# OpenGVLab/VisionLLM

Measured on NVIDIA H100. Metric: img_text_pairs_per_sec_fwd_1024px_256tok, higher is better.
Workload: dtype bf16

## Files before the change

visionllm_b200/csrc/gemm.cu:

```cuda
#include "common.cuh"
#include "tc_common.cuh"
#include "vllm_b200.h"

namespace {

constexpr int BM = 128, BK = 64, THREADS = 384, CONSUMER_WARPS = 8, CONSUMER_THREADS = CONSUMER_WARPS * 32;
constexpr int A_BYTES = BM * BK * 2;
constexpr int EPI_PITCH = 128 + 16;
constexpr int EPI_WARP_BYTES = 16 * EPI_PITCH;

enum { ACT_NONE = 0, ACT_GELU = 1, ACT_RELU = 2, ACT_SILU = 3, ACT_SWIGLU = 4, ACT_QUICKGELU = 5 };

struct GemmArgs {
  int M, N, K;
  void* C; int ldc;
  const __nv_bfloat16* bias; const __nv_bfloat16* colscale; const __nv_bfloat16* residual; int ldr;
  int act; int out_f32;
  const unsigned char* row_keep;
  int tiles_m, tiles_n;
  int group_m;
  int a_seg_kb, a_seg_rows;
  int sc_rows;
  void* sc_dst[8];
  uint32_t* sc_flag[8];
  int a_mn, b_mn;
  int bt_rows, causal;
};

struct TilePlan { int skip, kb0, kb1, b_row_off, k_off; };
__device__ __forceinline__ TilePlan plan_tile(const GemmArgs& g, int m0, int n0, int rows_per_tile, int num_kb) {
  TilePlan p{0, 0, num_kb, 0, 0};
  if (g.bt_rows) {
    const int bh = m0 / g.bt_rows, ml = m0 - bh * g.bt_rows;
    p.b_row_off = bh * g.N;
    p.k_off = bh * g.K;
    if (g.causal == 1 && n0 >= ml + rows_per_tile) p.skip = 1;
    if (g.causal == 2) p.kb0 = ml / BK;
    if (g.causal == 3) { const int e = (ml + rows_per_tile + BK - 1) / BK; p.kb1 = e < num_kb ? e : num_kb; }
  }
  return p;
}

template <int BN> struct Cfg {
  static constexpr int B_BYTES = BN * BK * 2;
  static constexpr int STAGE_BYTES = A_BYTES + B_BYTES;
  static constexpr int STAGES = BN == 256 ? 4 : 6;
  static constexpr int SMEM = STAGES * STAGE_BYTES + 1024  + 256  + 2 * BN * 4  +
                              CONSUMER_WARPS * EPI_WARP_BYTES ;
};

__device__ __forceinline__ float gelu_erf(float x) { return 0.5f * x * (1.f + erff(x * 0.70710678118654752f)); }
__device__ __forceinline__ float silu(float x) { return x / (1.f + __expf(-x)); }

__device__ __forceinline__ void tile_coords(int t, int tiles_m, int tiles_n, int group_m, int& tm, int& tn) {
  const int per_group = group_m * tiles_n;
  const int group = t / per_group;
  const int first = group * group_m;
  const int gsz = min(group_m, tiles_m - first);
  const int in = t - group * per_group;
  tm = first + in % gsz;
  tn = in / gsz;
}

template <int BN, int TA, int TB>
__device__ __forceinline__ void mma_kblock(float (&acc)[BN / 2], uint32_t sa, uint32_t sb, bool first_kb) {
  const uint64_t adesc = TA ? tc::wgmma_desc_sw128(sa, 8192, 1024) : tc::wgmma_desc_sw128(sa, 16, 1024);
  const uint64_t bdesc = TB ? tc::wgmma_desc_sw128(sb, 8192, 1024) : tc::wgmma_desc_sw128(sb, 16, 1024);
  constexpr uint64_t astep = TA ? 128 : 2, bstep = TB ? 128 : 2;
#pragma unroll
  for (int k = 0; k < BK / 16; ++k) {
    if constexpr (BN == 256)
      tc::wgmma_m64n256k16_ss<TA, TB>(acc, adesc + astep * k, bdesc + bstep * k, !(first_kb && k == 0));
    else
      tc::wgmma_m64n128k16_ss<TA, TB>(acc, adesc + astep * k, bdesc + bstep * k, !(first_kb && k == 0));
  }
}

enum { EPI_BF16 = 0, EPI_GENERAL = 1, EPI_SCATTER = 2 };

template <int BN, int TA, int TB, int EPI>
__global__ void __launch_bounds__(THREADS, 1)
gemm_bf16_wgmma_kernel(const __grid_constant__ CUtensorMap tmap_a, const __grid_constant__ CUtensorMap tmap_b,
                       const GemmArgs g) {
  using C_ = Cfg<BN>;
  constexpr int STAGES = C_::STAGES;
  extern __shared__ uint8_t smem_raw[];
  const uint32_t smem_base = (tc::smem_u32(smem_raw) + 1023u) & ~1023u;
  uint8_t* smem_gen = smem_raw + (smem_base - tc::smem_u32(smem_raw));
  const uint32_t bar_base = smem_base + STAGES * C_::STAGE_BYTES;
  auto full_bar = [&](int s) { return bar_base + 8 * s; };
  auto empty_bar = [&](int s) { return bar_base + 8 * (STAGES + s); };
  float* s_bias = reinterpret_cast<float*>(smem_gen + STAGES * C_::STAGE_BYTES + 256);
  float* s_scale = s_bias + BN;
  uint8_t* s_epi = reinterpret_cast<uint8_t*>(s_scale + BN);

  const int warp = threadIdx.x >> 5, lane = threadIdx.x & 31;
  const int n_tiles = g.tiles_m * g.tiles_n;
  const int num_kb = (g.K + BK - 1) / BK;

  if (warp == 0 && lane == 0) {
    tc::tma_prefetch_desc(&tmap_a);
    tc::tma_prefetch_desc(&tmap_b);
  }
  if (warp == 1 && lane == 0) {
    for (int s = 0; s < STAGES; ++s) { tc::mbar_init(full_bar(s), 1); tc::mbar_init(empty_bar(s), CONSUMER_WARPS); }
    tc::mbar_fence_init();
  }
  __syncthreads();

  if (warp < 4) {
    tc::reg_dealloc<40>();
    if (warp == 0 && tc::elect_one()) {
      int stage = 0; uint32_t phase = 0;
      for (int t = blockIdx.x; t < n_tiles; t += gridDim.x) {
        int tm, tn; tile_coords(t, g.tiles_m, g.tiles_n, g.group_m, tm, tn);
        const TilePlan tp = plan_tile(g, tm * BM, tn * BN, BM, num_kb);
        if (tp.skip) continue;
        const int bt_m0 = g.bt_rows ? (tm * BM) / g.bt_rows * g.bt_rows : 0;
        const int row_a = tm * BM - (TA ? bt_m0 : 0);
        const int row_b = tn * BN + (TB ? 0 : tp.b_row_off);
        const int ka_off = TA ? tp.k_off : 0, kb_off = TB ? tp.k_off : 0;
        for (int kb = tp.kb0; kb < tp.kb1; ++kb) {
          tc::mbar_wait(empty_bar(stage), phase ^ 1);
          const uint32_t sa = smem_base + stage * C_::STAGE_BYTES, sb = sa + A_BYTES;
          int ka = kb * BK + ka_off, ra = row_a;
          if (g.a_seg_kb) {
            const int seg = kb / g.a_seg_kb;
            ka = (kb - seg * g.a_seg_kb) * BK;
            ra = row_a + seg * g.a_seg_rows;
          }
          tc::mbar_arrive_expect_tx(full_bar(stage), C_::STAGE_BYTES);
          if constexpr (TA) {
            for (int h = 0; h < BM / 64; ++h) tc::tma_load_2d(sa + h * 8192, &tmap_a, full_bar(stage), ra + 64 * h, ka);
          } else {
            tc::tma_load_2d(sa, &tmap_a, full_bar(stage), ka, ra);
          }
          if constexpr (TB) {
            for (int h = 0; h < BN / 64; ++h)
              tc::tma_load_2d(sb + h * 8192, &tmap_b, full_bar(stage), row_b + 64 * h, kb * BK + kb_off);
          } else {
            tc::tma_load_2d(sb, &tmap_b, full_bar(stage), kb * BK, row_b);
          }
          if (++stage == STAGES) { stage = 0; phase ^= 1; }
        }
      }
    }
    return;
  }

  tc::reg_alloc<232>();
  const int wg = (warp - 4) >> 2;
  const int et = threadIdx.x - 128;
  const int frag_row = wg * 64 + (warp & 3) * 16 + (lane >> 2), frag_col = 2 * (lane & 3);
  const bool swiglu = EPI == EPI_GENERAL && g.act == ACT_SWIGLU;
  int stage = 0; uint32_t phase = 0;
  float acc[BN / 2];
  for (int t = blockIdx.x; t < n_tiles; t += gridDim.x) {
    int tm, tn; tile_coords(t, g.tiles_m, g.tiles_n, g.group_m, tm, tn);
    const TilePlan tp = plan_tile(g, tm * BM, tn * BN, BM, num_kb);
    if (tp.skip) continue;
    const int n0 = tn * BN;
    if (et < BN) {
      const int col = n0 + et;
      s_bias[et] = (g.bias && col < g.N) ? __bfloat162float(g.bias[col]) : 0.f;
      s_scale[et] = (g.colscale && col < g.N) ? __bfloat162float(g.colscale[col]) : 1.f;
    }
    int prev_stage = -1;
    for (int kb = tp.kb0; kb < tp.kb1; ++kb) {
      tc::mbar_wait(full_bar(stage), phase);
      const uint32_t sa = smem_base + stage * C_::STAGE_BYTES + wg * 8192, sb = smem_base + stage * C_::STAGE_BYTES + A_BYTES;
      const bool first = kb == tp.kb0;
      tc::acc_fence(acc);
      tc::wgmma_fence();
      mma_kblock<BN, TA, TB>(acc, sa, sb, first);
      tc::wgmma_commit();
      tc::wgmma_wait<1>();
      if (prev_stage >= 0 && lane == 0) tc::mbar_arrive(empty_bar(prev_stage));
      prev_stage = stage;
      if (++stage == STAGES) { stage = 0; phase ^= 1; }
    }
    tc::wgmma_wait<0>();
    tc::acc_fence(acc);
    if (lane == 0) tc::mbar_arrive(empty_bar(prev_stage));
    tc::named_bar_sync(1, CONSUMER_THREADS);

    auto math = [&](int row, int c, float& v0, float& v1) {
      const int col = n0 + c;
      v0 += s_bias[c]; v1 += s_bias[c + 1];
      if (g.act == ACT_GELU) { v0 = gelu_erf(v0); v1 = gelu_erf(v1); }
      else if (g.act == ACT_RELU) { v0 = fmaxf(v0, 0.f); v1 = fmaxf(v1, 0.f); }
      else if (g.act == ACT_SILU) { v0 = silu(v0); v1 = silu(v1); }
      else if (g.act == ACT_QUICKGELU) { v0 = v0 / (1.f + __expf(-1.702f * v0)); v1 = v1 / (1.f + __expf(-1.702f * v1)); }
      v0 *= s_scale[c]; v1 *= s_scale[c + 1];
      if (row >= g.M) return;
      if (g.residual) {
        const __nv_bfloat16* rp = g.residual + (size_t)row * g.ldr + col;
        if (col + 1 < g.N) {
          const float2 f = __bfloat1622float2(*reinterpret_cast<const __nv_bfloat162*>(rp));
          v0 += f.x; v1 += f.y;
        } else {
          v0 += __bfloat162float(rp[0]);
        }
      }
      if (g.row_keep && !g.row_keep[row]) { v0 = 0.f; v1 = 0.f; }
    };
    auto out_row = [&](int row) -> __nv_bfloat16* {
      if constexpr (EPI != EPI_SCATTER) return reinterpret_cast<__nv_bfloat16*>(g.C) + (size_t)row * g.ldc;
      const int d = row / g.sc_rows;
      return reinterpret_cast<__nv_bfloat16*>(g.sc_dst[d]) + (size_t)(row - d * g.sc_rows) * g.ldc;
    };
    auto emit = [&](int row, int c, float v0, float v1) {
      const int col = n0 + c;
      if (row >= g.M || col >= g.N) return;
      if (swiglu) {
        const int oc = col >> 1;
        float o = silu(v0 + s_bias[c]) * (v1 + s_bias[c + 1]);
        if (g.residual) o += __bfloat162float(g.residual[(size_t)row * g.ldr + oc]);
        reinterpret_cast<__nv_bfloat16*>(g.C)[(size_t)row * g.ldc + oc] = __float2bfloat16(o);
        return;
      }
      math(row, c, v0, v1);
      const bool pair = col + 1 < g.N;
      if (g.out_f32) {
        float* cp = reinterpret_cast<float*>(g.C) + (size_t)row * g.ldc + col;
        if (pair) *reinterpret_cast<float2*>(cp) = make_float2(v0, v1); else cp[0] = v0;
        return;
      }
      __nv_bfloat16* cp = out_row(row) + col;
      if (pair) *reinterpret_cast<__nv_bfloat162*>(cp) = __floats2bfloat162_rn(v0, v1); else cp[0] = __float2bfloat16(v0);
    };
    const int row0 = tm * BM + frag_row;
    const int warp_row0 = tm * BM + wg * 64 + (warp & 3) * 16;
    uint8_t* my_stage = s_epi + (warp - 4) * EPI_WARP_BYTES;
#pragma unroll
    for (int ch = 0; ch < BN / 64; ++ch) {
      const int c0 = ch * 64;
      if (n0 + c0 >= g.N) break;
      if constexpr (EPI == EPI_GENERAL) {
#pragma unroll
        for (int j = 8 * ch; j < 8 * ch + 8; ++j) {
          const int c = 8 * j + frag_col;
          emit(row0, c, acc[4 * j], acc[4 * j + 1]);
          emit(row0 + 8, c, acc[4 * j + 2], acc[4 * j + 3]);
        }
      } else {
#pragma unroll
        for (int j = 8 * ch; j < 8 * ch + 8; ++j) {
          const int c = 8 * j + frag_col;
          float a0 = acc[4 * j], a1 = acc[4 * j + 1], b0 = acc[4 * j + 2], b1 = acc[4 * j + 3];
          math(row0, c, a0, a1);
          math(row0 + 8, c, b0, b1);
          const int off = (8 * (j - 8 * ch) + frag_col) * 2;
          *reinterpret_cast<__nv_bfloat162*>(my_stage + (lane >> 2) * EPI_PITCH + off) = __floats2bfloat162_rn(a0, a1);
          *reinterpret_cast<__nv_bfloat162*>(my_stage + ((lane >> 2) + 8) * EPI_PITCH + off) = __floats2bfloat162_rn(b0, b1);
        }
        __syncwarp();
#pragma unroll
        for (int it = 0; it < 4; ++it) {
          const int rr = it * 4 + (lane >> 3), piece = lane & 7;
          const uint4 val = *reinterpret_cast<const uint4*>(my_stage + rr * EPI_PITCH + piece * 16);
          if (warp_row0 + rr < g.M) *reinterpret_cast<uint4*>(out_row(warp_row0 + rr) + n0 + c0 + piece * 8) = val;
        }
        __syncwarp();
      }
    }
    if constexpr (EPI == EPI_SCATTER) {
      __threadfence_system();
      __syncwarp();
      if (lane == 0 && warp_row0 < g.M)
        asm volatile("red.release.sys.global.add.u32 [%0], %1;" ::"l"(g.sc_flag[warp_row0 / g.sc_rows]), "r"(1u) : "memory");
    }
    tc::named_bar_sync(1, CONSUMER_THREADS);
  }
}

int g_sm_limit = 0, g_scatter_sm_limit = 0;

int g_gemm_variant = VLLM_GEMM_DEFAULT;

using KernelFn = void (*)(const CUtensorMap, const CUtensorMap, const GemmArgs);

template <int BN, int TA, int TB>
KernelFn pick_epilogue(const GemmArgs& g) {
  if (g.sc_rows) {
    if constexpr (BN == 256 && !TA && !TB) return gemm_bf16_wgmma_kernel<BN, TA, TB, EPI_SCATTER>;
    return nullptr;
  }
  if (g.act == ACT_SWIGLU || g.out_f32 || g.N % 64) return gemm_bf16_wgmma_kernel<BN, TA, TB, EPI_GENERAL>;
  return gemm_bf16_wgmma_kernel<BN, TA, TB, EPI_BF16>;
}
template <int BN>
KernelFn pick_kernel(const GemmArgs& g) {
  if (g.a_mn) return g.b_mn ? pick_epilogue<BN, 1, 1>(g) : pick_epilogue<BN, 1, 0>(g);
  return g.b_mn ? pick_epilogue<BN, 0, 1>(g) : pick_epilogue<BN, 0, 0>(g);
}

template <int BN>
int launch_gemm(const void* A, int lda, const void* B, int ldb, GemmArgs g, cudaStream_t st, long long a_rows = -1,
                int a_cols = -1) {
  using C_ = Cfg<BN>;
  CUtensorMap ta, tb;
  const uint64_t nb = g.bt_rows ? (uint64_t)(g.M / g.bt_rows) : 1;
  const uint64_t m_local = g.bt_rows ? (uint64_t)g.bt_rows : (uint64_t)g.M;
  int rc = g.a_mn ? vllm_make_tmap_bf16(&ta, A, nb * (uint64_t)g.K, m_local, (uint64_t)lda, 64)
                  : vllm_make_tmap_bf16(&ta, A, (uint64_t)(a_rows < 0 ? g.M : a_rows),
                                        (uint64_t)(a_cols < 0 ? g.K : a_cols), (uint64_t)lda, BM);
  if (rc) return rc;
  rc = g.b_mn ? vllm_make_tmap_bf16(&tb, B, nb * (uint64_t)g.K, (uint64_t)g.N, (uint64_t)ldb, 64)
              : vllm_make_tmap_bf16(&tb, B, nb * (uint64_t)g.N, (uint64_t)g.K, (uint64_t)ldb, BN);
  if (rc) return rc;
  g.tiles_m = (g.M + BM - 1) / BM;
  g.tiles_n = (g.N + BN - 1) / BN;
  const int n_tiles = g.tiles_m * g.tiles_n;
  int sms = vllm_num_sms();
  const int limit = g.sc_rows ? (g_scatter_sm_limit > 0 ? g_scatter_sm_limit : g_sm_limit) : g_sm_limit;
  if (limit > 0 && limit < sms) sms = limit;
  const int ctas = sms < n_tiles ? sms : n_tiles;
  g.group_m = 8;
  const KernelFn kern = pick_kernel<BN>(g);
  if (!kern) return VLLM_EUNSUPPORTED;
  const cudaError_t e = vllm_smem_optin(kern, C_::SMEM);
  if (e != cudaSuccess) return (int)e;
  kern<<<ctas, THREADS, C_::SMEM, st>>>(ta, tb, g);
  VLLM_CHECK_LAUNCH();
  return VLLM_OK;
}

bool wide_by_shape(const GemmArgs& g) {
  return !g.a_mn && !g.b_mn && !g.bt_rows && !g.a_seg_kb && g.N <= 4096 && g.K >= 3072;
}

int launch_gemm_auto(const void* A, int lda, const void* B, int ldb, const GemmArgs& g, cudaStream_t st, long long a_rows = -1,
                     int a_cols = -1) {
  const bool wide = g.sc_rows || g_gemm_variant == VLLM_GEMM_WIDE_TILE ||
                    (g_gemm_variant == VLLM_GEMM_DEFAULT && wide_by_shape(g));
  return wide ? launch_gemm<256>(A, lda, B, ldb, g, st, a_rows, a_cols) : launch_gemm<128>(A, lda, B, ldb, g, st, a_rows, a_cols);
}

}

extern "C" {

int vllm_gemm_set_variant(int v) {
  if (v != VLLM_GEMM_DEFAULT && v != VLLM_GEMM_WIDE_TILE && v != VLLM_GEMM_NARROW_TILE) return VLLM_EINVAL;
  g_gemm_variant = v;
  return VLLM_OK;
}
int vllm_gemm_set_sm_limit(int all_gemms, int scatter_gemm) {
  if (all_gemms < 0 || scatter_gemm < 0) return VLLM_EINVAL;
  g_sm_limit = all_gemms; g_scatter_sm_limit = scatter_gemm;
  return VLLM_OK;
}

static int gemm_bf16_common(const void* A, int lda, const void* B, int ldb, void* C, int ldc, int M, int N, int K,
                            const void* bias, const void* colscale, const void* residual, int ldr, int act, int out_f32,
                            const unsigned char* row_keep, void* stream);

int vllm_gemm_bf16(const void* A, int lda, const void* B, int ldb, void* C, int ldc, int M, int N, int K,
                   const void* bias, const void* colscale, const void* residual, int ldr, int act, int out_f32,
                   void* stream) {
  return gemm_bf16_common(A, lda, B, ldb, C, ldc, M, N, K, bias, colscale, residual, ldr, act, out_f32, nullptr, stream);
}

int vllm_gemm_bf16_rowmask(const void* A, int lda, const void* B, int ldb, void* C, int ldc, int M, int N, int K,
                           const void* bias, const void* colscale, const void* residual, int ldr, int act, int out_f32,
                           const unsigned char* row_keep, void* stream) {
  if (!row_keep || act == ACT_SWIGLU) return VLLM_EINVAL;
  return gemm_bf16_common(A, lda, B, ldb, C, ldc, M, N, K, bias, colscale, residual, ldr, act, out_f32, row_keep, stream);
}

static int gemm_bf16_common(const void* A, int lda, const void* B, int ldb, void* C, int ldc, int M, int N, int K,
                            const void* bias, const void* colscale, const void* residual, int ldr, int act, int out_f32,
                            const unsigned char* row_keep, void* stream) {
  if (M < 0 || N <= 0 || K <= 0 || lda < K || ldb < K) return VLLM_EINVAL;
  if (M == 0) return VLLM_OK;
  if (!A || !B || !C) return VLLM_EINVAL;
  if (act < 0 || act > ACT_QUICKGELU) return VLLM_EINVAL;
  const int n_out = act == ACT_SWIGLU ? N / 2 : N;
  if (act == ACT_SWIGLU && (N % 2 || out_f32 || colscale)) return VLLM_EUNSUPPORTED;
  if (ldc < n_out || (residual && ldr < n_out)) return VLLM_EINVAL;
  if (!vllm_aligned(A, 16) || !vllm_aligned(B, 16) || (lda % 8) || (ldb % 8)) return VLLM_EALIGN;
  const int celt = out_f32 ? 4 : 2;
  if (!vllm_aligned(C, 16) || ((size_t)ldc * celt) % 16 || (residual && (!vllm_aligned(residual, 16) || ldr % 8)))
    return VLLM_EALIGN;
  GemmArgs g{};
  g.M = M; g.N = N; g.K = K; g.C = C; g.ldc = ldc;
  g.bias = (const __nv_bfloat16*)bias; g.colscale = (const __nv_bfloat16*)colscale;
  g.residual = (const __nv_bfloat16*)residual; g.ldr = ldr; g.act = act; g.out_f32 = out_f32;
  g.row_keep = row_keep;
  cudaStream_t st = (cudaStream_t)stream;
  return launch_gemm_auto(A, lda, B, ldb, g, st);
}

int vllm_gemm_bf16_tn(const void* A, int lda, int a_mn_major, const void* B, int ldb, int b_mn_major, void* C, int ldc, int M,
                      int N, int K, int out_f32, void* stream) {
  if (M < 0 || N <= 0 || K <= 0) return VLLM_EINVAL;
  if (M == 0) return VLLM_OK;
  if (!A || !B || !C) return VLLM_EINVAL;
  if (lda < (a_mn_major ? M : K) || ldb < (b_mn_major ? N : K) || ldc < N) return VLLM_EINVAL;
  if (!vllm_aligned(A, 16) || !vllm_aligned(B, 16) || (lda % 8) || (ldb % 8)) return VLLM_EALIGN;
  if (!vllm_aligned(C, 16) || ((size_t)ldc * (out_f32 ? 4 : 2)) % 16) return VLLM_EALIGN;
  GemmArgs g{};
  g.M = M; g.N = N; g.K = K; g.C = C; g.ldc = ldc; g.out_f32 = out_f32;
  g.a_mn = a_mn_major ? 1 : 0; g.b_mn = b_mn_major ? 1 : 0;
  cudaStream_t st = (cudaStream_t)stream;
  return launch_gemm_auto(A, lda, B, ldb, g, st);
}

int vllm_gemm_bf16_batched(const void* A, int lda, int a_mn_major, const void* B, int ldb, int b_mn_major, void* C, int ldc,
                           int n_batch, int M, int N, int K, int causal, int out_f32, void* stream) {
  if (n_batch < 0 || M <= 0 || N <= 0 || K <= 0 || causal < 0 || causal > 3) return VLLM_EINVAL;
  if (causal >= 2 && K != M) return VLLM_EINVAL;
// ... 59 lines not shown
```

visionllm_b200/csrc/tc_common.cuh:

```cuda
#pragma once
#include <cuda.h>
#include <cuda_runtime.h>
#include <stdint.h>

namespace tc {

__device__ __forceinline__ uint32_t smem_u32(const void* p) {
  return static_cast<uint32_t>(__cvta_generic_to_shared(p));
}
__device__ __forceinline__ bool elect_one() {
  uint32_t pred = 0;
  asm volatile(
      "{\n\t.reg .pred P;\n\telect.sync _|P, 0xffffffff;\n\tselp.u32 %0, 1, 0, P;\n\t}\n"
      : "=r"(pred));
  return pred != 0;
}

__device__ __forceinline__ void mbar_init(uint32_t bar, uint32_t count) {
  asm volatile("mbarrier.init.shared::cta.b64 [%0], %1;" ::"r"(bar), "r"(count) : "memory");
}
__device__ __forceinline__ void mbar_fence_init() {
  asm volatile("fence.mbarrier_init.release.cluster;" ::: "memory");
}
__device__ __forceinline__ void mbar_arrive_expect_tx(uint32_t bar, uint32_t bytes) {
  asm volatile("mbarrier.arrive.expect_tx.shared::cta.b64 _, [%0], %1;" ::"r"(bar), "r"(bytes) : "memory");
}
__device__ __forceinline__ void mbar_arrive(uint32_t bar) {
  asm volatile("mbarrier.arrive.shared::cta.b64 _, [%0];" ::"r"(bar) : "memory");
}
__device__ __forceinline__ bool mbar_try_wait(uint32_t bar, uint32_t parity) {
  uint32_t ok;
  asm volatile(
      "{\n\t.reg .pred p;\n\tmbarrier.try_wait.parity.shared::cta.b64 p, [%1], %2;\n\tselp.u32 %0, 1, 0, p;\n\t}\n"
      : "=r"(ok)
      : "r"(bar), "r"(parity)
      : "memory");
  return ok != 0;
}
__device__ __forceinline__ void mbar_wait(uint32_t bar, uint32_t parity) {
  while (!mbar_try_wait(bar, parity)) {
  }
}
__device__ __forceinline__ void tma_prefetch_desc(const CUtensorMap* m) {
  asm volatile("prefetch.tensormap [%0];" ::"l"(reinterpret_cast<uint64_t>(m)) : "memory");
}
__device__ __forceinline__ void tma_load_2d(uint32_t dst, const CUtensorMap* m, uint32_t bar, int c0, int c1) {
  asm volatile(
      "cp.async.bulk.tensor.2d.shared::cluster.global.mbarrier::complete_tx::bytes [%0], [%1, {%3, %4}], [%2];" ::"r"(dst),
      "l"(reinterpret_cast<uint64_t>(m)), "r"(bar), "r"(c0), "r"(c1)
      : "memory");
}

template <int N> __device__ __forceinline__ void reg_dealloc() { asm volatile("setmaxnreg.dec.sync.aligned.u32 %0;" ::"n"(N)); }
template <int N> __device__ __forceinline__ void reg_alloc() { asm volatile("setmaxnreg.inc.sync.aligned.u32 %0;" ::"n"(N)); }
__device__ __forceinline__ void named_bar_sync(int id, int threads) {
  asm volatile("bar.sync %0, %1;" ::"r"(id), "r"(threads) : "memory");
}

__device__ __forceinline__ void wgmma_fence() { asm volatile("wgmma.fence.sync.aligned;" ::: "memory"); }
__device__ __forceinline__ void wgmma_commit() { asm volatile("wgmma.commit_group.sync.aligned;" ::: "memory"); }
template <int N> __device__ __forceinline__ void wgmma_wait() { asm volatile("wgmma.wait_group.sync.aligned %0;" ::"n"(N) : "memory"); }
template <int N> __device__ __forceinline__ void acc_fence(float (&d)[N]) {
#pragma unroll
  for (int i = 0; i < N; ++i) asm volatile("" : "+f"(d[i])::"memory");
}

template <int TA, int TB>
__device__ __forceinline__ void wgmma_m64n128k16_ss(float (&d)[64], uint64_t adesc, uint64_t bdesc, uint32_t accumulate) {
  asm volatile(
      "{\n\t.reg .pred p;\n\tsetp.ne.b32 p, %66, 0;\n\t"
      "wgmma.mma_async.sync.aligned.m64n128k16.f32.bf16.bf16 {"
      "%0, %1, %2, %3, %4, %5, %6, %7, %8, %9, %10, %11, %12, %13, %14, %15, %16, %17, %18, %19, %20, %21, "
      "%22, %23, %24, %25, %26, %27, %28, %29, %30, %31, %32, %33, %34, %35, %36, %37, %38, %39, %40, %41, "
      "%42, %43, %44, %45, %46, %47, %48, %49, %50, %51, %52, %53, %54, %55, %56, %57, %58, %59, %60, %61, "
      "%62, %63 "
      "}, %64, %65, p, 1, 1, %67, %68;\n\t}\n"
      : "+f"(d[0]), "+f"(d[1]), "+f"(d[2]), "+f"(d[3]), "+f"(d[4]), "+f"(d[5]), "+f"(d[6]), "+f"(d[7]),
        "+f"(d[8]), "+f"(d[9]), "+f"(d[10]), "+f"(d[11]), "+f"(d[12]), "+f"(d[13]), "+f"(d[14]), "+f"(d[15]),
        "+f"(d[16]), "+f"(d[17]), "+f"(d[18]), "+f"(d[19]), "+f"(d[20]), "+f"(d[21]), "+f"(d[22]), "+f"(d[23]),
        "+f"(d[24]), "+f"(d[25]), "+f"(d[26]), "+f"(d[27]), "+f"(d[28]), "+f"(d[29]), "+f"(d[30]), "+f"(d[31]),
        "+f"(d[32]), "+f"(d[33]), "+f"(d[34]), "+f"(d[35]), "+f"(d[36]), "+f"(d[37]), "+f"(d[38]), "+f"(d[39]),
        "+f"(d[40]), "+f"(d[41]), "+f"(d[42]), "+f"(d[43]), "+f"(d[44]), "+f"(d[45]), "+f"(d[46]), "+f"(d[47]),
        "+f"(d[48]), "+f"(d[49]), "+f"(d[50]), "+f"(d[51]), "+f"(d[52]), "+f"(d[53]), "+f"(d[54]), "+f"(d[55]),
        "+f"(d[56]), "+f"(d[57]), "+f"(d[58]), "+f"(d[59]), "+f"(d[60]), "+f"(d[61]), "+f"(d[62]), "+f"(d[63])
      : "l"(adesc), "l"(bdesc), "r"(accumulate), "n"(TA), "n"(TB));
}
template <int TA, int TB>
__device__ __forceinline__ void wgmma_m64n256k16_ss(float (&d)[128], uint64_t adesc, uint64_t bdesc, uint32_t accumulate) {
  asm volatile(
      "{\n\t.reg .pred p;\n\tsetp.ne.b32 p, %130, 0;\n\t"
      "wgmma.mma_async.sync.aligned.m64n256k16.f32.bf16.bf16 {"
      "%0, %1, %2, %3, %4, %5, %6, %7, %8, %9, %10, %11, %12, %13, %14, %15, %16, %17, %18, %19, %20, %21, "
      "%22, %23, %24, %25, %26, %27, %28, %29, %30, %31, %32, %33, %34, %35, %36, %37, %38, %39, %40, %41, %42, %43, "
      "%44, %45, %46, %47, %48, %49, %50, %51, %52, %53, %54, %55, %56, %57, %58, %59, %60, %61, %62, %63, %64, %65, "
      "%66, %67, %68, %69, %70, %71, %72, %73, %74, %75, %76, %77, %78, %79, %80, %81, %82, %83, %84, %85, %86, %87, "
      "%88, %89, %90, %91, %92, %93, %94, %95, %96, %97, %98, %99, %100, %101, %102, %103, %104, %105, %106, %107, %108, %109, "
      "%110, %111, %112, %113, %114, %115, %116, %117, %118, %119, %120, %121, %122, %123, %124, %125, %126, %127 "
      "}, %128, %129, p, 1, 1, %131, %132;\n\t}\n"
      : "+f"(d[0]), "+f"(d[1]), "+f"(d[2]), "+f"(d[3]), "+f"(d[4]), "+f"(d[5]), "+f"(d[6]), "+f"(d[7]),
        "+f"(d[8]), "+f"(d[9]), "+f"(d[10]), "+f"(d[11]), "+f"(d[12]), "+f"(d[13]), "+f"(d[14]), "+f"(d[15]),
        "+f"(d[16]), "+f"(d[17]), "+f"(d[18]), "+f"(d[19]), "+f"(d[20]), "+f"(d[21]), "+f"(d[22]), "+f"(d[23]),
        "+f"(d[24]), "+f"(d[25]), "+f"(d[26]), "+f"(d[27]), "+f"(d[28]), "+f"(d[29]), "+f"(d[30]), "+f"(d[31]),
        "+f"(d[32]), "+f"(d[33]), "+f"(d[34]), "+f"(d[35]), "+f"(d[36]), "+f"(d[37]), "+f"(d[38]), "+f"(d[39]),
        "+f"(d[40]), "+f"(d[41]), "+f"(d[42]), "+f"(d[43]), "+f"(d[44]), "+f"(d[45]), "+f"(d[46]), "+f"(d[47]),
        "+f"(d[48]), "+f"(d[49]), "+f"(d[50]), "+f"(d[51]), "+f"(d[52]), "+f"(d[53]), "+f"(d[54]), "+f"(d[55]),
        "+f"(d[56]), "+f"(d[57]), "+f"(d[58]), "+f"(d[59]), "+f"(d[60]), "+f"(d[61]), "+f"(d[62]), "+f"(d[63]),
        "+f"(d[64]), "+f"(d[65]), "+f"(d[66]), "+f"(d[67]), "+f"(d[68]), "+f"(d[69]), "+f"(d[70]), "+f"(d[71]),
        "+f"(d[72]), "+f"(d[73]), "+f"(d[74]), "+f"(d[75]), "+f"(d[76]), "+f"(d[77]), "+f"(d[78]), "+f"(d[79]),
        "+f"(d[80]), "+f"(d[81]), "+f"(d[82]), "+f"(d[83]), "+f"(d[84]), "+f"(d[85]), "+f"(d[86]), "+f"(d[87]),
        "+f"(d[88]), "+f"(d[89]), "+f"(d[90]), "+f"(d[91]), "+f"(d[92]), "+f"(d[93]), "+f"(d[94]), "+f"(d[95]),
        "+f"(d[96]), "+f"(d[97]), "+f"(d[98]), "+f"(d[99]), "+f"(d[100]), "+f"(d[101]), "+f"(d[102]), "+f"(d[103]),
        "+f"(d[104]), "+f"(d[105]), "+f"(d[106]), "+f"(d[107]), "+f"(d[108]), "+f"(d[109]), "+f"(d[110]), "+f"(d[111]),
        "+f"(d[112]), "+f"(d[113]), "+f"(d[114]), "+f"(d[115]), "+f"(d[116]), "+f"(d[117]), "+f"(d[118]), "+f"(d[119]),
        "+f"(d[120]), "+f"(d[121]), "+f"(d[122]), "+f"(d[123]), "+f"(d[124]), "+f"(d[125]), "+f"(d[126]), "+f"(d[127])
      : "l"(adesc), "l"(bdesc), "r"(accumulate), "n"(TA), "n"(TB));
}
__device__ __forceinline__ void wgmma_m64n64k16_ss(float (&d)[32], uint64_t adesc, uint64_t bdesc, uint32_t accumulate) {
  asm volatile(
      "{\n\t.reg .pred p;\n\tsetp.ne.b32 p, %34, 0;\n\t"
      "wgmma.mma_async.sync.aligned.m64n64k16.f32.bf16.bf16 {"
      "%0, %1, %2, %3, %4, %5, %6, %7, %8, %9, %10, %11, %12, %13, %14, %15, %16, %17, %18, %19, %20, %21, "
      "%22, %23, %24, %25, %26, %27, %28, %29, %30, %31 "
      "}, %32, %33, p, 1, 1, 0, 0;\n\t}\n"
      : "+f"(d[0]), "+f"(d[1]), "+f"(d[2]), "+f"(d[3]), "+f"(d[4]), "+f"(d[5]), "+f"(d[6]), "+f"(d[7]),
        "+f"(d[8]), "+f"(d[9]), "+f"(d[10]), "+f"(d[11]), "+f"(d[12]), "+f"(d[13]), "+f"(d[14]), "+f"(d[15]),
        "+f"(d[16]), "+f"(d[17]), "+f"(d[18]), "+f"(d[19]), "+f"(d[20]), "+f"(d[21]), "+f"(d[22]), "+f"(d[23]),
        "+f"(d[24]), "+f"(d[25]), "+f"(d[26]), "+f"(d[27]), "+f"(d[28]), "+f"(d[29]), "+f"(d[30]), "+f"(d[31])
      : "l"(adesc), "l"(bdesc), "r"(accumulate));
}
__device__ __forceinline__ void wgmma_m64n128k16_rs(float (&d)[64], const uint32_t (&a)[4], uint64_t bdesc, uint32_t accumulate) {
  asm volatile(
      "{\n\t.reg .pred p;\n\tsetp.ne.b32 p, %69, 0;\n\t"
      "wgmma.mma_async.sync.aligned.m64n128k16.f32.bf16.bf16 {"
      "%0, %1, %2, %3, %4, %5, %6, %7, %8, %9, %10, %11, %12, %13, %14, %15, %16, %17, %18, %19, %20, %21, "
      "%22, %23, %24, %25, %26, %27, %28, %29, %30, %31, %32, %33, %34, %35, %36, %37, %38, %39, %40, %41, "
      "%42, %43, %44, %45, %46, %47, %48, %49, %50, %51, %52, %53, %54, %55, %56, %57, %58, %59, %60, %61, "
      "%62, %63 "
      "}, {%64, %65, %66, %67}, %68, p, 1, 1, 1;\n\t}\n"
      : "+f"(d[0]), "+f"(d[1]), "+f"(d[2]), "+f"(d[3]), "+f"(d[4]), "+f"(d[5]), "+f"(d[6]), "+f"(d[7]),
        "+f"(d[8]), "+f"(d[9]), "+f"(d[10]), "+f"(d[11]), "+f"(d[12]), "+f"(d[13]), "+f"(d[14]), "+f"(d[15]),
        "+f"(d[16]), "+f"(d[17]), "+f"(d[18]), "+f"(d[19]), "+f"(d[20]), "+f"(d[21]), "+f"(d[22]), "+f"(d[23]),
        "+f"(d[24]), "+f"(d[25]), "+f"(d[26]), "+f"(d[27]), "+f"(d[28]), "+f"(d[29]), "+f"(d[30]), "+f"(d[31]),
        "+f"(d[32]), "+f"(d[33]), "+f"(d[34]), "+f"(d[35]), "+f"(d[36]), "+f"(d[37]), "+f"(d[38]), "+f"(d[39]),
        "+f"(d[40]), "+f"(d[41]), "+f"(d[42]), "+f"(d[43]), "+f"(d[44]), "+f"(d[45]), "+f"(d[46]), "+f"(d[47]),
        "+f"(d[48]), "+f"(d[49]), "+f"(d[50]), "+f"(d[51]), "+f"(d[52]), "+f"(d[53]), "+f"(d[54]), "+f"(d[55]),
        "+f"(d[56]), "+f"(d[57]), "+f"(d[58]), "+f"(d[59]), "+f"(d[60]), "+f"(d[61]), "+f"(d[62]), "+f"(d[63])
      : "r"(a[0]), "r"(a[1]), "r"(a[2]), "r"(a[3]), "l"(bdesc), "r"(accumulate));
}

__device__ __forceinline__ uint64_t wgmma_desc_sw128(uint32_t smem_addr, uint32_t lbo_bytes, uint32_t sbo_bytes) {
  uint64_t d = 0;
  d |= (uint64_t)((smem_addr & 0x3FFFF) >> 4);
  d |= (uint64_t)(lbo_bytes >> 4) << 16;
  d |= (uint64_t)(sbo_bytes >> 4) << 32;
  d |= (uint64_t)1 << 62;
  return d;
}

}

#include <cudaTypedefs.h>
static inline PFN_cuTensorMapEncodeTiled_v12000 vllm_tma_encoder() {
  static PFN_cuTensorMapEncodeTiled_v12000 fn = nullptr;
  if (!fn) {
    void* p = nullptr;
    cudaDriverEntryPointQueryResult q;
    if (cudaGetDriverEntryPoint("cuTensorMapEncodeTiled", &p, cudaEnableDefault, &q) == cudaSuccess &&
        q == cudaDriverEntryPointSuccess)
      fn = reinterpret_cast<PFN_cuTensorMapEncodeTiled_v12000>(p);
  }
  return fn;
}
static inline int vllm_make_tmap_bf16(CUtensorMap* m, const void* base, uint64_t rows, uint64_t cols, uint64_t ld,
                                      uint32_t box_rows) {
  PFN_cuTensorMapEncodeTiled_v12000 enc = vllm_tma_encoder();
  if (!enc) return -100;
  cuuint64_t dims[2] = {cols, rows};
  cuuint64_t strides[1] = {ld * 2};
  cuuint32_t box[2] = {64, box_rows};
  cuuint32_t estr[2] = {1, 1};
  CUresult r = enc(m, CU_TENSOR_MAP_DATA_TYPE_BFLOAT16, 2, const_cast<void*>(base), dims, strides, box, estr,
                   CU_TENSOR_MAP_INTERLEAVE_NONE, CU_TENSOR_MAP_SWIZZLE_128B, CU_TENSOR_MAP_L2_PROMOTION_L2_256B,
                   CU_TENSOR_MAP_FLOAT_OOB_FILL_NONE);
  return r == CUDA_SUCCESS ? 0 : -101;
}
```

Before: 5.973.

## Move GEMM epilogue to TMA stores with prefetched residual tiles and specialized variants

Rewrites the GEMM epilogue so each consumer warp stages its output in swizzled double-buffered shared memory and writes it with TMA bulk tensor stores. Residual tiles are prefetched by TMA ahead of use, and bias, scale and row_keep vectors are loaded with cp.async instead of per-thread loads. SwiGLU and fp32 outputs get their own specialized epilogue variants in place of the general scalar path, and the wide-tile heuristic now triggers on N >= 2048. This adds more shared memory, extra mbarriers and bulk-group synchronisation. It also drops SwiGLU support for transposed operands.

New measurement: 7.072, median of 6. +18.4%, better.

```diff
diff --git a/visionllm_b200/csrc/gemm.cu b/visionllm_b200/csrc/gemm.cu
--- a/visionllm_b200/csrc/gemm.cu
+++ b/visionllm_b200/csrc/gemm.cu
@@ -6,8 +6,8 @@
 
 constexpr int BM = 128, BK = 64, THREADS = 384, CONSUMER_WARPS = 8, CONSUMER_THREADS = CONSUMER_WARPS * 32;
 constexpr int A_BYTES = BM * BK * 2;
-constexpr int EPI_PITCH = 128 + 16;
-constexpr int EPI_WARP_BYTES = 16 * EPI_PITCH;
+constexpr int EPI_BUF = 16 * 128;
+constexpr int SMEM_LIMIT = 232448;
 
 enum { ACT_NONE = 0, ACT_GELU = 1, ACT_RELU = 2, ACT_SILU = 3, ACT_SWIGLU = 4, ACT_QUICKGELU = 5 };
 
@@ -45,8 +45,14 @@
   static constexpr int B_BYTES = BN * BK * 2;
   static constexpr int STAGE_BYTES = A_BYTES + B_BYTES;
   static constexpr int STAGES = BN == 256 ? 4 : 6;
-  static constexpr int SMEM = STAGES * STAGE_BYTES + 1024  + 256  + 2 * BN * 4  +
-                              CONSUMER_WARPS * EPI_WARP_BYTES ;
+  static constexpr int EPI_OFF = STAGES * STAGE_BYTES;
+  static constexpr int BAR_OFF = EPI_OFF + CONSUMER_WARPS * 2 * EPI_BUF;
+  static constexpr int BIAS_OFF = BAR_OFF + 256;
+  static constexpr int SCALE_OFF = BIAS_OFF + 2 * BN + 4;
+  static constexpr int KEEP_OFF = SCALE_OFF + 2 * BN + 4;
+  static constexpr int SMEM = 1024  + KEEP_OFF + BM + 4;
+  static_assert(8 * (2 * STAGES + 2 * CONSUMER_WARPS) <= 256, "mbarriers overflow their slot");
+  static_assert(SMEM <= SMEM_LIMIT, "shared memory over the per-block limit");
 };
 
 __device__ __forceinline__ float gelu_erf(float x) { return 0.5f * x * (1.f + erff(x * 0.70710678118654752f)); }
@@ -76,23 +82,24 @@
   }
 }
 
-enum { EPI_BF16 = 0, EPI_GENERAL = 1, EPI_SCATTER = 2 };
+enum { EPI_BF16 = 0, EPI_SWIGLU = 1, EPI_F32 = 2, EPI_SCATTER = 3 };
+
+__device__ __forceinline__ int swz(int r, int b) { return r * 128 + ((((b >> 4) ^ r) & 7) << 4) + (b & 15); }
 
 template <int BN, int TA, int TB, int EPI>
 __global__ void __launch_bounds__(THREADS, 1)
 gemm_bf16_wgmma_kernel(const __grid_constant__ CUtensorMap tmap_a, const __grid_constant__ CUtensorMap tmap_b,
+                       const __grid_constant__ CUtensorMap tmap_c, const __grid_constant__ CUtensorMap tmap_r,
                        const GemmArgs g) {
   using C_ = Cfg<BN>;
   constexpr int STAGES = C_::STAGES;
   extern __shared__ uint8_t smem_raw[];
   const uint32_t smem_base = (tc::smem_u32(smem_raw) + 1023u) & ~1023u;
   uint8_t* smem_gen = smem_raw + (smem_base - tc::smem_u32(smem_raw));
-  const uint32_t bar_base = smem_base + STAGES * C_::STAGE_BYTES;
+  const uint32_t bar_base = smem_base + C_::BAR_OFF;
   auto full_bar = [&](int s) { return bar_base + 8 * s; };
   auto empty_bar = [&](int s) { return bar_base + 8 * (STAGES + s); };
-  float* s_bias = reinterpret_cast<float*>(smem_gen + STAGES * C_::STAGE_BYTES + 256);
-  float* s_scale = s_bias + BN;
-  uint8_t* s_epi = reinterpret_cast<uint8_t*>(s_scale + BN);
+  auto res_bar = [&](int i) { return bar_base + 8 * (2 * STAGES + i); };
 
   const int warp = threadIdx.x >> 5, lane = threadIdx.x & 31;
   const int n_tiles = g.tiles_m * g.tiles_n;
@@ -101,9 +108,14 @@
   if (warp == 0 && lane == 0) {
     tc::tma_prefetch_desc(&tmap_a);
     tc::tma_prefetch_desc(&tmap_b);
+    if constexpr (EPI != EPI_SCATTER) {
+      tc::tma_prefetch_desc(&tmap_c);
+      if (g.residual) tc::tma_prefetch_desc(&tmap_r);
+    }
   }
   if (warp == 1 && lane == 0) {
     for (int s = 0; s < STAGES; ++s) { tc::mbar_init(full_bar(s), 1); tc::mbar_init(empty_bar(s), CONSUMER_WARPS); }
+    for (int i = 0; i < 2 * CONSUMER_WARPS; ++i) tc::mbar_init(res_bar(i), 1);
     tc::mbar_fence_init();
   }
   __syncthreads();
@@ -150,9 +162,26 @@
 
   tc::reg_alloc<232>();
   const int wg = (warp - 4) >> 2;
+  const int cw = warp - 4;
   const int et = threadIdx.x - 128;
-  const int frag_row = wg * 64 + (warp & 3) * 16 + (lane >> 2), frag_col = 2 * (lane & 3);
-  const bool swiglu = EPI == EPI_GENERAL && g.act == ACT_SWIGLU;
+  const int lr = lane >> 2, frag_col = 2 * (lane & 3);
+  const bool has_res = EPI != EPI_SCATTER && g.residual != nullptr;
+  constexpr int UNIT_COLS = EPI == EPI_SWIGLU ? 128 : 64;
+  constexpr int UNITS = BN / UNIT_COLS;
+  constexpr int RES_AHEAD = EPI == EPI_F32 ? 1 : 2;
+  const int n_out = EPI == EPI_SWIGLU ? g.N / 2 : g.N;
+  uint8_t* s_buf = smem_gen + C_::EPI_OFF + cw * 2 * EPI_BUF;
+  const uint32_t s_buf_u32 = smem_base + C_::EPI_OFF + cw * 2 * EPI_BUF;
+  const uint32_t s_bias = smem_base + C_::BIAS_OFF, s_scale = smem_base + C_::SCALE_OFF, s_keep = smem_base + C_::KEEP_OFF;
+  const __nv_bfloat16* bias_t = reinterpret_cast<const __nv_bfloat16*>(smem_gen + C_::BIAS_OFF + (reinterpret_cast<uintptr_t>(g.bias) & 3));
+  const __nv_bfloat16* scale_t =
+      reinterpret_cast<const __nv_bfloat16*>(smem_gen + C_::SCALE_OFF + (reinterpret_cast<uintptr_t>(g.colscale) & 3));
+  const uint8_t* keep_t = smem_gen + C_::KEEP_OFF + (reinterpret_cast<uintptr_t>(g.row_keep) & 3);
+  if (et <= BN / 2) {
+    if (!g.bias) *reinterpret_cast<uint32_t*>(smem_gen + C_::BIAS_OFF + 4 * et) = 0u;
+    if (!g.colscale) *reinterpret_cast<uint32_t*>(smem_gen + C_::SCALE_OFF + 4 * et) = 0x3F803F80u;
+  }
+  uint32_t res_phase = 0;
   int stage = 0; uint32_t phase = 0;
   float acc[BN / 2];
   for (int t = blockIdx.x; t < n_tiles; t += gridDim.x) {
@@ -160,10 +189,22 @@
     const TilePlan tp = plan_tile(g, tm * BM, tn * BN, BM, num_kb);
     if (tp.skip) continue;
     const int n0 = tn * BN;
-    if (et < BN) {
-      const int col = n0 + et;
-      s_bias[et] = (g.bias && col < g.N) ? __bfloat162float(g.bias[col]) : 0.f;
-      s_scale[et] = (g.colscale && col < g.N) ? __bfloat162float(g.colscale[col]) : 1.f;
+    const int oc0 = EPI == EPI_SWIGLU ? n0 / 2 : n0;
+    const int warp_row0 = tm * BM + cw * 16;
+    const bool warp_live = warp_row0 < g.M;
+    if (g.bias && et <= BN / 2) tc::cp_async_vec_word(s_bias, g.bias, 2LL * g.N, 2LL * n0, et);
+    if (g.colscale && et <= BN / 2) tc::cp_async_vec_word(s_scale, g.colscale, 2LL * g.N, 2LL * n0, et);
+    if (g.row_keep && et <= BM / 4) tc::cp_async_vec_word(s_keep, g.row_keep, g.M, (long long)tm * BM, et);
+    auto load_res = [&](int u) {
+      const int b = EPI == EPI_F32 ? 0 : (u & 1);
+      tc::mbar_arrive_expect_tx(res_bar(2 * cw + b), EPI_BUF);
+      tc::tma_load_2d(s_buf_u32 + b * EPI_BUF, &tmap_r, res_bar(2 * cw + b), oc0 + 64 * u, warp_row0);
+    };
+    if (has_res && warp_live && lane == 0) {
+      tc::bulk_wait_read<0>();
+#pragma unroll
+      for (int u = 0; u < RES_AHEAD && u < UNITS; ++u)
+        if (oc0 + 64 * u < n_out) load_res(u);
     }
     int prev_stage = -1;
     for (int kb = tp.kb0; kb < tp.kb1; ++kb) {
@@ -182,103 +223,164 @@
     tc::wgmma_wait<0>();
     tc::acc_fence(acc);
     if (lane == 0) tc::mbar_arrive(empty_bar(prev_stage));
+    tc::cp_async_wait_all();
     tc::named_bar_sync(1, CONSUMER_THREADS);
 
-    auto math = [&](int row, int c, float& v0, float& v1) {
-      const int col = n0 + c;
-      v0 += s_bias[c]; v1 += s_bias[c + 1];
-      if (g.act == ACT_GELU) { v0 = gelu_erf(v0); v1 = gelu_erf(v1); }
-      else if (g.act == ACT_RELU) { v0 = fmaxf(v0, 0.f); v1 = fmaxf(v1, 0.f); }
-      else if (g.act == ACT_SILU) { v0 = silu(v0); v1 = silu(v1); }
-      else if (g.act == ACT_QUICKGELU) { v0 = v0 / (1.f + __expf(-1.702f * v0)); v1 = v1 / (1.f + __expf(-1.702f * v1)); }
-      v0 *= s_scale[c]; v1 *= s_scale[c + 1];
-      if (row >= g.M) return;
-      if (g.residual) {
-        const __nv_bfloat16* rp = g.residual + (size_t)row * g.ldr + col;
-        if (col + 1 < g.N) {
-          const float2 f = __bfloat1622float2(*reinterpret_cast<const __nv_bfloat162*>(rp));
-          v0 += f.x; v1 += f.y;
-        } else {
-          v0 += __bfloat162float(rp[0]);
+#pragma unroll
+    for (int j = 0; j < BN / 8; ++j) {
+      const int c = 8 * j + frag_col;
+      const float b0 = __bfloat162float(bias_t[c]), b1 = __bfloat162float(bias_t[c + 1]);
+      acc[4 * j] = __fadd_rn(acc[4 * j], b0); acc[4 * j + 1] = __fadd_rn(acc[4 * j + 1], b1);
+      acc[4 * j + 2] = __fadd_rn(acc[4 * j + 2], b0); acc[4 * j + 3] = __fadd_rn(acc[4 * j + 3], b1);
+    }
+    if constexpr (EPI == EPI_BF16 || EPI == EPI_F32) {
+      switch (g.act) {
+        case ACT_GELU:
+#pragma unroll
+          for (int i = 0; i < BN / 2; ++i) acc[i] = gelu_erf(acc[i]);
+          break;
+        case ACT_RELU:
+#pragma unroll
+          for (int i = 0; i < BN / 2; ++i) acc[i] = fmaxf(acc[i], 0.f);
+          break;
+        case ACT_SILU:
+#pragma unroll
+          for (int i = 0; i < BN / 2; ++i) acc[i] = silu(acc[i]);
+          break;
+        case ACT_QUICKGELU:
+#pragma unroll
+          for (int i = 0; i < BN / 2; ++i) acc[i] = acc[i] / (1.f + __expf(-1.702f * acc[i]));
+          break;
+        default: break;
+      }
+    }
+    bool keep0 = true, keep1 = true;
+    if (g.row_keep) { keep0 = keep_t[cw * 16 + lr] != 0; keep1 = keep_t[cw * 16 + lr + 8] != 0; }
+
+    constexpr int E = EPI == EPI_F32 ? 4 : 2;
+    auto put_box = [&](int bi, int col0) {
+      if ((n_out * E) % 16 == 0 || col0 + 128 / E <= n_out) {
+        if (lane == 0) tc::tma_store_2d(&tmap_c, s_buf_u32 + bi * EPI_BUF, col0, warp_row0);
+        return;
+      }
+#pragma unroll
+      for (int it = 0; it < 4; ++it) {
+        const int rr = it * 4 + (lane >> 3), piece = lane & 7, row = warp_row0 + rr;
+        if (row >= g.M) continue;
+#pragma unroll
+        for (int e = 0; e < 16 / E; ++e) {
+          const int col = col0 + piece * (16 / E) + e;
+          if (col >= n_out) break;
+          const uint8_t* sp = s_buf + bi * EPI_BUF + swz(rr, 16 * piece + E * e);
+          uint8_t* dp = reinterpret_cast<uint8_t*>(g.C) + ((size_t)row * g.ldc + col) * E;
+          if constexpr (E == 4) *reinterpret_cast<uint32_t*>(dp) = *reinterpret_cast<const uint32_t*>(sp);
+          else *reinterpret_cast<uint16_t*>(dp) = *reinterpret_cast<const uint16_t*>(sp);
         }
       }
-      if (g.row_keep && !g.row_keep[row]) { v0 = 0.f; v1 = 0.f; }
     };
-    auto out_row = [&](int row) -> __nv_bfloat16* {
-      if constexpr (EPI != EPI_SCATTER) return reinterpret_cast<__nv_bfloat16*>(g.C) + (size_t)row * g.ldc;
-      const int d = row / g.sc_rows;
-      return reinterpret_cast<__nv_bfloat16*>(g.sc_dst[d]) + (size_t)(row - d * g.sc_rows) * g.ldc;
-    };
-    auto emit = [&](int row, int c, float v0, float v1) {
-      const int col = n0 + c;
-      if (row >= g.M || col >= g.N) return;
-      if (swiglu) {
-        const int oc = col >> 1;
-        float o = silu(v0 + s_bias[c]) * (v1 + s_bias[c + 1]);
-        if (g.residual) o += __bfloat162float(g.residual[(size_t)row * g.ldr + oc]);
-        reinterpret_cast<__nv_bfloat16*>(g.C)[(size_t)row * g.ldc + oc] = __float2bfloat16(o);
-        return;
-      }
-      math(row, c, v0, v1);
-      const bool pair = col + 1 < g.N;
-      if (g.out_f32) {
-        float* cp = reinterpret_cast<float*>(g.C) + (size_t)row * g.ldc + col;
-        if (pair) *reinterpret_cast<float2*>(cp) = make_float2(v0, v1); else cp[0] = v0;
-        return;
-      }
-      __nv_bfloat16* cp = out_row(row) + col;
-      if (pair) *reinterpret_cast<__nv_bfloat162*>(cp) = __floats2bfloat162_rn(v0, v1); else cp[0] = __float2bfloat16(v0);
-    };
-    const int row0 = tm * BM + frag_row;
-    const int warp_row0 = tm * BM + wg * 64 + (warp & 3) * 16;
-    uint8_t* my_stage = s_epi + (warp - 4) * EPI_WARP_BYTES;
-#pragma unroll
-    for (int ch = 0; ch < BN / 64; ++ch) {
-      const int c0 = ch * 64;
-      if (n0 + c0 >= g.N) break;
-      if constexpr (EPI == EPI_GENERAL) {
-#pragma unroll
-        for (int j = 8 * ch; j < 8 * ch + 8; ++j) {
-          const int c = 8 * j + frag_col;
-          emit(row0, c, acc[4 * j], acc[4 * j + 1]);
-          emit(row0 + 8, c, acc[4 * j + 2], acc[4 * j + 3]);
+
+    if (warp_live) {
+#pragma unroll
+      for (int u = 0; u < UNITS; ++u) {
+        if (oc0 + 64 * u >= n_out) break;
+        const int b = EPI == EPI_F32 ? 0 : (u & 1);
+        uint8_t* buf = s_buf + b * EPI_BUF;
+        if (has_res) {
+          if (u > 0 && u + RES_AHEAD - 1 < UNITS && oc0 + 64 * (u + RES_AHEAD - 1) < n_out && lane == 0) {
+            tc::bulk_wait_read<0>();
+            load_res(u + RES_AHEAD - 1);
+          }
+          tc::mbar_wait(res_bar(2 * cw + b), (res_phase >> b) & 1);
+          res_phase ^= 1u << b;
+        } else if constexpr (EPI != EPI_SCATTER && EPI != EPI_F32) {
+          if (lane == 0) { if (u == 0) tc::bulk_wait_read<0>(); else tc::bulk_wait_read<1>(); }
+          __syncwarp();
         }
-      } else {
-#pragma unroll
-        for (int j = 8 * ch; j < 8 * ch + 8; ++j) {
-          const int c = 8 * j + frag_col;
-          float a0 = acc[4 * j], a1 = acc[4 * j + 1], b0 = acc[4 * j + 2], b1 = acc[4 * j + 3];
-          math(row0, c, a0, a1);
-          math(row0 + 8, c, b0, b1);
-          const int off = (8 * (j - 8 * ch) + frag_col) * 2;
-          *reinterpret_cast<__nv_bfloat162*>(my_stage + (lane >> 2) * EPI_PITCH + off) = __floats2bfloat162_rn(a0, a1);
-          *reinterpret_cast<__nv_bfloat162*>(my_stage + ((lane >> 2) + 8) * EPI_PITCH + off) = __floats2bfloat162_rn(b0, b1);
+        if constexpr (EPI == EPI_SWIGLU) {
+#pragma unroll
+          for (int jj = 0; jj < 16; ++jj) {
+            const int j = 16 * u + jj;
+#pragma unroll
+            for (int h = 0; h < 2; ++h) {
+              uint8_t* p = buf + swz(lr + 8 * h, 16 * (jj >> 1)) + 8 * (jj & 1) + 2 * (lane & 3);
+              float o = __fmul_rn(silu(acc[4 * j + 2 * h]), acc[4 * j + 2 * h + 1]);
+              if (has_res) o = __fadd_rn(o, __bfloat162float(*reinterpret_cast<const __nv_bfloat16*>(p)));
+              *reinterpret_cast<__nv_bfloat16*>(p) = __float2bfloat16(o);
+            }
+          }
+        } else {
+#pragma unroll
+          for (int jj = 0; jj < 8; ++jj) {
+            const int j = 8 * u + jj, c = 8 * j + frag_col;
+            const float s0 = __bfloat162float(scale_t[c]), s1 = __bfloat162float(scale_t[c + 1]);
+#pragma unroll
+            for (int h = 0; h < 2; ++h) {
+              float& v0 = acc[4 * j + 2 * h];
+              float& v1 = acc[4 * j + 2 * h + 1];
+              uint8_t* p = buf + swz(lr + 8 * h, 16 * jj) + 4 * (lane & 3);
+              v0 = __fmul_rn(v0, s0); v1 = __fmul_rn(v1, s1);
+              if (has_res) {
+                const float2 f = __bfloat1622float2(*reinterpret_cast<const __nv_bfloat162*>(p));
+                v0 = __fadd_rn(v0, f.x); v1 = __fadd_rn(v1, f.y);
+              }
+              if (!(h ? keep1 : keep0)) { v0 = 0.f; v1 = 0.f; }
+              if constexpr (EPI != EPI_F32) *reinterpret_cast<__nv_bfloat162*>(p) = __floats2bfloat162_rn(v0, v1);
+            }
+          }
+          if constexpr (EPI == EPI_F32) {
+            if (lane == 0) tc::bulk_wait_read<0>();
+            __syncwarp();
+#pragma unroll
+            for (int jj = 0; jj < 8; ++jj) {
+              const int j = 8 * u + jj;
+#pragma unroll
+              for (int h = 0; h < 2; ++h) {
+                uint8_t* p = s_buf + (jj >> 2) * EPI_BUF + swz(lr + 8 * h, 32 * (jj & 3) + 8 * (lane & 3));
+                *reinterpret_cast<float2*>(p) = make_float2(acc[4 * j + 2 * h], acc[4 * j + 2 * h + 1]);
+              }
+            }
+          }
         }
-        __syncwarp();
-#pragma unroll
-        for (int it = 0; it < 4; ++it) {
-          const int rr = it * 4 + (lane >> 3), piece = lane & 7;
-          const uint4 val = *reinterpret_cast<const uint4*>(my_stage + rr * EPI_PITCH + piece * 16);
-          if (warp_row0 + rr < g.M) *reinterpret_cast<uint4*>(out_row(warp_row0 + rr) + n0 + c0 + piece * 8) = val;
+        if constexpr (EPI == EPI_SCATTER) {
+          __syncwarp();
+          const int d = warp_row0 / g.sc_rows;
+          __nv_bfloat16* dst = reinterpret_cast<__nv_bfloat16*>(g.sc_dst[d]) + (size_t)(warp_row0 - d * g.sc_rows) * g.ldc + n0 + 64 * u;
+#pragma unroll
+          for (int it = 0; it < 4; ++it) {
+            const int rr = it * 4 + (lane >> 3), piece = lane & 7;
+            const uint4 val = *reinterpret_cast<const uint4*>(buf + swz(rr, 16 * piece));
+            *reinterpret_cast<uint4*>(dst + (size_t)rr * g.ldc + piece * 8) = val;
+          }
+          __syncwarp();
+        } else {
+          tc::fence_proxy_async_smem();
+          __syncwarp();
+          if constexpr (EPI == EPI_F32) {
+            put_box(0, n0 + 64 * u);
+            if (n0 + 64 * u + 32 < n_out) put_box(1, n0 + 64 * u + 32);
+          } else {
+            put_box(b, oc0 + 64 * u);
+          }
+          if (lane == 0) tc::bulk_commit();
         }
-        __syncwarp();
       }
     }
     if constexpr (EPI == EPI_SCATTER) {
       __threadfence_system();
       __syncwarp();
-      if (lane == 0 && warp_row0 < g.M)
+      if (lane == 0 && warp_live)
         asm volatile("red.release.sys.global.add.u32 [%0], %1;" ::"l"(g.sc_flag[warp_row0 / g.sc_rows]), "r"(1u) : "memory");
     }
     tc::named_bar_sync(1, CONSUMER_THREADS);
   }
+  if (EPI != EPI_SCATTER && lane == 0) tc::bulk_wait<0>();
 }
 
 int g_sm_limit = 0, g_scatter_sm_limit = 0;
 
 int g_gemm_variant = VLLM_GEMM_DEFAULT;
 
-using KernelFn = void (*)(const CUtensorMap, const CUtensorMap, const GemmArgs);
+using KernelFn = void (*)(const CUtensorMap, const CUtensorMap, const CUtensorMap, const CUtensorMap, const GemmArgs);
 
 template <int BN, int TA, int TB>
 KernelFn pick_epilogue(const GemmArgs& g) {
@@ -286,7 +388,11 @@
     if constexpr (BN == 256 && !TA && !TB) return gemm_bf16_wgmma_kernel<BN, TA, TB, EPI_SCATTER>;
     return nullptr;
   }
-  if (g.act == ACT_SWIGLU || g.out_f32 || g.N % 64) return gemm_bf16_wgmma_kernel<BN, TA, TB, EPI_GENERAL>;
+  if (g.act == ACT_SWIGLU) {
+    if constexpr (!TA && !TB) return gemm_bf16_wgmma_kernel<BN, TA, TB, EPI_SWIGLU>;
+    return nullptr;
+  }
+  if (g.out_f32) return gemm_bf16_wgmma_kernel<BN, TA, TB, EPI_F32>;
   return gemm_bf16_wgmma_kernel<BN, TA, TB, EPI_BF16>;
 }
 template <int BN>
@@ -302,13 +408,20 @@
   CUtensorMap ta, tb;
   const uint64_t nb = g.bt_rows ? (uint64_t)(g.M / g.bt_rows) : 1;
   const uint64_t m_local = g.bt_rows ? (uint64_t)g.bt_rows : (uint64_t)g.M;
-  int rc = g.a_mn ? vllm_make_tmap_bf16(&ta, A, nb * (uint64_t)g.K, m_local, (uint64_t)lda, 64)
-                  : vllm_make_tmap_bf16(&ta, A, (uint64_t)(a_rows < 0 ? g.M : a_rows),
+  int rc = g.a_mn ? vllm_make_tmap_2d(&ta, A, nb * (uint64_t)g.K, m_local, (uint64_t)lda, 64)
+                  : vllm_make_tmap_2d(&ta, A, (uint64_t)(a_rows < 0 ? g.M : a_rows),
                                         (uint64_t)(a_cols < 0 ? g.K : a_cols), (uint64_t)lda, BM);
   if (rc) return rc;
-  rc = g.b_mn ? vllm_make_tmap_bf16(&tb, B, nb * (uint64_t)g.K, (uint64_t)g.N, (uint64_t)ldb, 64)
-              : vllm_make_tmap_bf16(&tb, B, nb * (uint64_t)g.N, (uint64_t)g.K, (uint64_t)ldb, BN);
+  rc = g.b_mn ? vllm_make_tmap_2d(&tb, B, nb * (uint64_t)g.K, (uint64_t)g.N, (uint64_t)ldb, 64)
+              : vllm_make_tmap_2d(&tb, B, nb * (uint64_t)g.N, (uint64_t)g.K, (uint64_t)ldb, BN);
   if (rc) return rc;
+  CUtensorMap tc_{}, tr{};
+  if (!g.sc_rows) {
+    const uint64_t n_out = (uint64_t)(g.act == ACT_SWIGLU ? g.N / 2 : g.N);
+    rc = vllm_make_tmap_2d(&tc_, g.C, (uint64_t)g.M, n_out, (uint64_t)g.ldc, 16, g.out_f32 != 0);
+    if (!rc && g.residual) rc = vllm_make_tmap_2d(&tr, g.residual, (uint64_t)g.M, n_out, (uint64_t)g.ldr, 16);
+    if (rc) return rc;
+  }
   g.tiles_m = (g.M + BM - 1) / BM;
   g.tiles_n = (g.N + BN - 1) / BN;
   const int n_tiles = g.tiles_m * g.tiles_n;
@@ -321,13 +434,13 @@
   if (!kern) return VLLM_EUNSUPPORTED;
   const cudaError_t e = vllm_smem_optin(kern, C_::SMEM);
   if (e != cudaSuccess) return (int)e;
-  kern<<<ctas, THREADS, C_::SMEM, st>>>(ta, tb, g);
+  kern<<<ctas, THREADS, C_::SMEM, st>>>(ta, tb, tc_, tr, g);
   VLLM_CHECK_LAUNCH();
   return VLLM_OK;
 }
 
 bool wide_by_shape(const GemmArgs& g) {
-  return !g.a_mn && !g.b_mn && !g.bt_rows && !g.a_seg_kb && g.N <= 4096 && g.K >= 3072;
+  return !g.a_mn && !g.b_mn && !g.bt_rows && !g.a_seg_kb && g.N >= 2048;
 }
 
 int launch_gemm_auto(const void* A, int lda, const void* B, int ldb, const GemmArgs& g, cudaStream_t st, long long a_rows = -1,
diff --git a/visionllm_b200/csrc/tc_common.cuh b/visionllm_b200/csrc/tc_common.cuh
--- a/visionllm_b200/csrc/tc_common.cuh
+++ b/visionllm_b200/csrc/tc_common.cuh
@@ -50,6 +50,24 @@
       "l"(reinterpret_cast<uint64_t>(m)), "r"(bar), "r"(c0), "r"(c1)
       : "memory");
 }
+__device__ __forceinline__ void tma_store_2d(const CUtensorMap* m, uint32_t src, int c0, int c1) {
+  asm volatile("cp.async.bulk.tensor.2d.global.shared::cta.bulk_group [%0, {%2, %3}], [%1];" ::"l"(reinterpret_cast<uint64_t>(m)),
+               "r"(src), "r"(c0), "r"(c1)
+               : "memory");
+}
+__device__ __forceinline__ void bulk_commit() { asm volatile("cp.async.bulk.commit_group;" ::: "memory"); }
+template <int N> __device__ __forceinline__ void bulk_wait_read() { asm volatile("cp.async.bulk.wait_group.read %0;" ::"n"(N) : "memory"); }
+template <int N> __device__ __forceinline__ void bulk_wait() { asm volatile("cp.async.bulk.wait_group %0;" ::"n"(N) : "memory"); }
+__device__ __forceinline__ void fence_proxy_async_smem() { asm volatile("fence.proxy.async.shared::cta;" ::: "memory"); }
+
+__device__ __forceinline__ void cp_async_vec_word(uint32_t dst, const void* v, long long len, long long b0, int i) {
+  const uintptr_t base = reinterpret_cast<uintptr_t>(v);
+  const uintptr_t w = ((base + b0) & ~uintptr_t(3)) + 4u * i;
+  const long long left = (long long)(base + len) - (long long)w;
+  const int n = left >= 4 ? 4 : left > 0 ? (int)left : 0;
+  asm volatile("cp.async.ca.shared.global [%0], [%1], 4, %2;" ::"r"(dst + 4u * i), "l"(w), "r"(n) : "memory");
+}
+__device__ __forceinline__ void cp_async_wait_all() { asm volatile("cp.async.wait_all;" ::: "memory"); }
 
 template <int N> __device__ __forceinline__ void reg_dealloc() { asm volatile("setmaxnreg.dec.sync.aligned.u32 %0;" ::"n"(N)); }
 template <int N> __device__ __forceinline__ void reg_alloc() { asm volatile("setmaxnreg.inc.sync.aligned.u32 %0;" ::"n"(N)); }
@@ -171,16 +189,17 @@
   }
   return fn;
 }
-static inline int vllm_make_tmap_bf16(CUtensorMap* m, const void* base, uint64_t rows, uint64_t cols, uint64_t ld,
-                                      uint32_t box_rows) {
+static inline int vllm_make_tmap_2d(CUtensorMap* m, const void* base, uint64_t rows, uint64_t cols, uint64_t ld,
+                                    uint32_t box_rows, bool f32 = false) {
   PFN_cuTensorMapEncodeTiled_v12000 enc = vllm_tma_encoder();
   if (!enc) return -100;
+  const uint32_t elt = f32 ? 4 : 2;
   cuuint64_t dims[2] = {cols, rows};
-  cuuint64_t strides[1] = {ld * 2};
-  cuuint32_t box[2] = {64, box_rows};
+  cuuint64_t strides[1] = {ld * elt};
+  cuuint32_t box[2] = {128 / elt, box_rows};
   cuuint32_t estr[2] = {1, 1};
-  CUresult r = enc(m, CU_TENSOR_MAP_DATA_TYPE_BFLOAT16, 2, const_cast<void*>(base), dims, strides, box, estr,
-                   CU_TENSOR_MAP_INTERLEAVE_NONE, CU_TENSOR_MAP_SWIZZLE_128B, CU_TENSOR_MAP_L2_PROMOTION_L2_256B,
-                   CU_TENSOR_MAP_FLOAT_OOB_FILL_NONE);
+  CUresult r = enc(m, f32 ? CU_TENSOR_MAP_DATA_TYPE_FLOAT32 : CU_TENSOR_MAP_DATA_TYPE_BFLOAT16, 2, const_cast<void*>(base),
+                   dims, strides, box, estr, CU_TENSOR_MAP_INTERLEAVE_NONE, CU_TENSOR_MAP_SWIZZLE_128B,
+                   CU_TENSOR_MAP_L2_PROMOTION_L2_256B, CU_TENSOR_MAP_FLOAT_OOB_FILL_NONE);
   return r == CUDA_SUCCESS ? 0 : -101;
 }
```
